# nichmorgan/better-search-rag-rust

Hardware: AMD Instinct MI355X
Metric: queries/sec + p50 latency, 768-d top-10 over N vectors @1/2/4/8 GPU (higher is better)
Workload: dtype f32; 1 GPU; configs[2]: 10M x 768 f32 corpus sharded over the N GPUs, 1000 batched queries, top-10; rows_total=10000000, rows_per_gpu_rank0=10000000, queries=1000, top_k=10, dim=768, parallelism=corpus sharded over 1 GPU(s) (interval_by_rank)

## Files before the change

### better-search-rag-rust_amd/csrc/index.cpp

```cpp
#include <math.h>
#include <stdio.h>
#include <string.h>
#include <time.h>

#include <algorithm>

#include "internal.hpp"
#include "kernels.hpp"

namespace bsr {

constexpr uint32_t kMaxKForFilter = 200;

static thread_local std::string g_err;

int set_error(int code, const char* fmt, ...) {
    char buf[1024];
    va_list ap;
    va_start(ap, fmt);
    vsnprintf(buf, sizeof buf, fmt, ap);
    va_end(ap);
    g_err = buf;
    return code;
}
// ... 632 lines not shown
                (unsigned long long)live, (unsigned long long)first, t1 - t0, t2 - t1, host_ms() - t2);
    return BSR_OK;
}

int bsr_index_compact_impl(bsr_index* ix, uint64_t new_global_offset, uint32_t flags, uint64_t* out_old_ids,
                           uint64_t out_capacity, uint64_t* out_count) {
    if (!ix) return set_error(BSR_E_INVALID, "null index");
    return ix->compact_rows(new_global_offset, flags, out_old_ids, out_capacity, out_count);
}

static int run_exact_scan(bsr_index* ix, const int32_t* ids, uint32_t n_ids, uint32_t k) {
    if (!n_ids) return BSR_OK;
    const uint32_t groups = (n_ids + kScanQF - 1) / kScanQF;
    const uint32_t grid = scan_grid_for(ix->n);
    BSR_TRY(ix->part.ensure((size_t)grid * kScanQF * k * sizeof(uint64_t)));
    ev_begin(ix, ix->ev_scan, 1);
    for (uint32_t g = 0; g < groups; ++g) {
        const uint32_t nqf = std::min(kScanQF, n_ids - g * kScanQF);
        const int32_t* qid = ids + (size_t)g * kScanQF;
        BSR_HIP(launch_scan_exact(ix->rows.as<float>(), ix->ld, ix->dim, ix->n, ix->na.as<float>(),
                                  ix->qf32.as<float>(), qid, nqf, ix->nb.as<float>(), k, grid,
                                  ix->part.as<uint64_t>(), ix->stream));
        BSR_HIP(launch_merge_parts(ix->part.as<uint64_t>(), grid, qid, nqf, k, ix->keys.as<uint64_t>(), ix->stream));
    }
    ev_end(ix, ix->ev_scan);
    return BSR_OK;
}

static int run_list_scan(bsr_index* ix, const int32_t* ids, uint32_t n_ids, uint32_t k, const uint32_t* list,
                         uint32_t n_list);
static int run_exact_rounds(bsr_index* ix, const int32_t* ids, uint32_t n_ids, uint32_t k) {
    if (!ix->n_dead) return run_exact_scan(ix, ids, n_ids, k);
    BSR_TRY(ix->ensure_live_list());
    return run_list_scan(ix, ids, n_ids, k, ix->live_list.as<uint32_t>(), (uint32_t)ix->live_rows());
}

static uint32_t top_slots(const bsr_index* ix, uint32_t nq, uint32_t k) {
    const char* v = getenv("BSR_SKINNY_TOP");
    if (v && v[0] == '0') return 0;
    if (nq > kSkinnyMaxQ || ix->n < kSkinnyTopMinRows || kp_for(k) > 63 || k > 64 || ix->op_row_bytes > 16 * 64 ||
        ix->ld % 64 != 0 || ix->ld > 1024 || !rescore_kp_enabled())
        return 0;
    const uint32_t slots = 4 * skinny_top_lists((uint32_t)ix->n);
    return slots <= 64u * kTopKeysPerLane ? slots : 0;
}

static int filter_buffers(bsr_index* ix, uint32_t nq, uint32_t qpad, uint32_t k, uint32_t cap_in = 0) {
    const uint32_t kp = kp_for(k);
    const uint32_t cap = std::max(cap_in ? cap_in : cap_for(k), top_slots(ix, nq, k));
    ix->stats.n_candidates = kp;
    BSR_TRY(ix->tau.ensure((size_t)qpad * sizeof(float)));
    BSR_TRY(ix->cand.ensure((size_t)qpad * cap * sizeof(uint64_t)));
    BSR_TRY(ix->cnt.ensure(((size_t)qpad + 8 * kTailCounters + kGangWords) * sizeof(uint32_t)));
    BSR_TRY(ix->cand_rows.ensure((size_t)nq * kp * sizeof(uint32_t)));
    BSR_TRY(ix->ncand.ensure((size_t)nq * sizeof(uint32_t)));
    BSR_TRY(ix->tau_excl.ensure((size_t)nq * sizeof(float)));
    BSR_TRY(ix->fail.ensure((size_t)nq * sizeof(uint32_t)));
    BSR_TRY(ix->fail2.ensure((size_t)nq * sizeof(uint32_t)));
    return BSR_OK;
}

static GemmArgs gemm_args(bsr_index* ix, uint32_t qpad) {
    GemmArgs g{};
    g.A = ix->fop.as<uint8_t>();
    g.B = ix->qop.as<uint8_t>();
    g.row_bytes = ix->op_row_bytes;
    g.n_qt = qpad / kFilterTile;
    g.a_scale = ix->ascale.as<float>();
    g.b_scale = ix->qscale.as<float>();
    return g;
}
static GemmArgs emit_args(bsr_index* ix, uint32_t nq, uint32_t qpad) {
    GemmArgs g = gemm_args(ix, qpad);
    g.a_stride = ix->op_row_bytes;
    g.a_scale_rows = kQuantBlock;
    g.n_rows = (uint32_t)ix->n;
    g.n_rt = (uint32_t)((ix->n + kFilterTile - 1) / kFilterTile);
    g.cand = ix->cand.as<uint64_t>();
    g.cnt = ix->cnt.as<uint32_t>();
    g.n_q = nq;
    return g;
}

struct SampleLayout {
    uint32_t n_s, n_rt_s;
    bool compact;
    uint32_t tiles;
    uint32_t s_ld, n_vals;
};
static bool sample_tiles_on() {
    const char* v = getenv("BSR_SAMPLE_TILES");
    return !(v && v[0] == '0');
}
static SampleLayout sample_layout(const bsr_index* ix, uint32_t nq, uint32_t ks) {
    SampleLayout L{};
    const uint32_t BM = kFilterTile;
    L.n_s = (uint32_t)((ix->n + kSampleStride - 1) / kSampleStride);
    L.n_rt_s = (L.n_s + BM - 1) / BM;
    L.compact = L.n_s >= 32u * 8u * ks;
    const uint32_t nk = ix->op_row_bytes / 64;
    const bool qs16 = ix->op_row_bytes % 64 == 0 && nk % 2 == 0 && nk >= 2 && nk <= 12;
    if (L.compact && nq > kSkinnyMaxQ && qs16 && sample_tiles_on()) L.tiles = sample_tiles_for(ix->n);
    if (L.tiles) {
        const uint64_t last0 = ((uint64_t)(L.tiles - 1) * kSampleTileEvery + kSampleTilePhase) * 128;
        const uint64_t valid = std::min<uint64_t>(128, ix->n - last0);
        L.s_ld = 4 * L.tiles;
        L.n_vals = 4 * (L.tiles - 1) + (uint32_t)((valid + kQuantBlock - 1) / kQuantBlock);
    } else {
        L.s_ld = L.compact ? L.n_rt_s * (BM / 32) : L.n_rt_s * BM;
        L.n_vals = L.compact ? (L.n_s + 31) / 32 : L.n_s;
    }
    return L;
}

static int sample_pass(bsr_index* ix, uint32_t nq, uint32_t qpad, uint32_t k, uint64_t* smax, uint32_t ks_in = 0,
                       uint32_t cap_in = 0, const uint32_t* ks_q = nullptr) {
    BSR_TRY(filter_buffers(ix, nq, qpad, k, cap_in));
    ix->smp_tiles = 0;
    const bool skinny = nq <= kSkinnyMaxQ;
    const uint32_t cap = cap_in ? cap_in : cap_for(k);
    const uint32_t ks = ks_in ? ks_in : ks_for(k);
    const uint64_t n = ix->n;
    GemmArgs g = gemm_args(ix, qpad);
    uint32_t* status = ix->d_status;
    if (n > cap) {
        const SampleLayout L = sample_layout(ix, nq, ks);
        const uint32_t s_ld = L.s_ld, n_vals = L.n_vals;
        BSR_TRY(ix->S.ensure((size_t)qpad * s_ld * sizeof(float)));
        g.a_stride = ix->op_row_bytes;
        if (L.tiles) {
            g.a_scale_rows = kQuantBlock;
            g.n_rows = (uint32_t)n;
            g.n_rt = L.tiles;
            g.s_tiles = L.tiles;
            g.s_vals = n_vals;
            ix->smp_tiles = L.tiles;
            ix->smp_ld = s_ld;
            ix->smp_vals = n_vals;
        } else {
            g.A = ix->fop_s.as<uint8_t>();
            g.a_scale = ix->ascale_s.as<float>();
            g.a_scale_rows = kSampleScaleRows;
            g.n_rows = L.n_s;
            g.n_rt = L.n_rt_s;
        }
        g.S = ix->S.as<float>();
        g.s_ld = s_ld;
        g.s_compact = L.compact ? 1u : 0u;
        BSR_HIP(launch_timed(ix, ix->ev_sample, [&] {
            return skinny ? launch_filter_skinny_sample(g, ix->stream) : launch_filter_sample(g, ix->stream);
        }, 2));
        BSR_HIP(launch_select_tau(ix->S.as<float>(), s_ld, n_vals, nq, qpad, ix->qflags.as<uint32_t>(), ks,
                                  ix->tau.as<float>(), ix->cnt.as<uint32_t>(), status, ix->stream, smax, ks_q));
    } else {
        BSR_HIP(launch_select_tau(nullptr, 0, 0, nq, qpad, ix->qflags.as<uint32_t>(), ks, ix->tau.as<float>(),
                                  ix->cnt.as<uint32_t>(), status, ix->stream, smax, ks_q));
    }
    return BSR_OK;
}

static int emit_pass(bsr_index* ix, uint32_t nq, uint32_t qpad, uint32_t k, uint32_t cap_in = 0) {
    const bool skinny = nq <= kSkinnyMaxQ;
    GemmArgs g = emit_args(ix, nq, qpad);
    g.tau = ix->tau.as<float>();
    g.cap = cap_in ? cap_in : cap_for(k);
    g.tail = g.n_qt <= kTailCounters ? ix->cnt.as<uint32_t>() + qpad : nullptr;
    g.s_tiles = skinny ? 0u : ix->smp_tiles;
    g.S = ix->S.as<float>();
    g.s_ld = ix->smp_ld;
    g.s_vals = ix->smp_vals;
    BSR_HIP(launch_timed(ix, ix->ev_emit, [&] {
        hipError_t r = skinny ? launch_filter_skinny_emit(g, ix->stream) : launch_filter_emit(g, ix->stream);
        if (r == hipSuccess && g.s_tiles) r = launch_sample_fixup(g, ix->stream);
        return r;
    }));
    return BSR_OK;
}

static uint32_t top_layout_lab() {
    const char* lay = getenv("BSR_TOP_LAYOUT");
    return lay && lay[0] == '0' ? 0u : 2u;
}

static int top_pass(bsr_index* ix, uint32_t nq, uint32_t qpad, uint32_t k, uint32_t top) {
    BSR_TRY(filter_buffers(ix, nq, qpad, k));
    GemmArgs g = emit_args(ix, nq, qpad);
    g.cap = top;
    g.status = ix->d_status;
// ... 892 lines not shown
```

### better-search-rag-rust_amd/csrc/internal.hpp

```cpp
#pragma once

#include <hip/hip_runtime.h>
#include <stdarg.h>
#include <stdint.h>

#include <atomic>

#include <string>
#include <vector>

#include "bsr.h"
#include "kernels.hpp"

namespace bsr {

int set_error(int code, const char* fmt, ...);
void clear_error();

#define BSR_HIP(call)                                                                       \
    do {                                                                                    \
        hipError_t e_ = (call);                                                             \
        if (e_ != hipSuccess)                                                               \
            return ::bsr::set_error(BSR_E_HIP, "%s failed: %s (%s:%d)", #call,              \
                                    hipGetErrorString(e_), __FILE__, __LINE__);             \
// ... 5 lines not shown
        if (r_ != BSR_OK) return r_; \
    } while (0)

extern std::atomic<uint64_t> g_alloc_gen;

struct DevBuf {
    void* p = nullptr;
    size_t bytes = 0;
    int ensure(size_t need);
    void release();
    template <class T> T* as() const { return static_cast<T*>(p); }
    ~DevBuf() { release(); }
};

bool is_device_ptr(const void* p);
void* coherent_host_alias(const void* p);
hipError_t stream_wait(hipStream_t s);
hipError_t flag_wait(const uint32_t* flag, hipStream_t s);
int select_device(int device);

static inline uint64_t round_up(uint64_t x, uint64_t m) { return (x + m - 1) / m * m; }

struct Events {
    hipEvent_t a = nullptr, b = nullptr;
    bool armed = false;
    ~Events();
    int create();
};

}

struct bsr_index {
    bsr_config cfg{};
    int device = 0;
    hipStream_t stream = nullptr;
    uint32_t dim = 0, ld = 0;
    uint64_t n = 0, n_pad = 0, global_offset = 0;
    bool loaded = false;
    bool approx_ok = false;
    uint32_t row_flags = 0;
    uint32_t op_row_bytes = 0;
    float row_ebound = 0.0f;

    bsr::DevBuf rows;
    bsr::DevBuf na;
    bsr::DevBuf fop;
    bsr::DevBuf fop_s;
    bsr::DevBuf ascale_s;
    uint32_t smp_tiles = 0, smp_ld = 0, smp_vals = 0;
    bsr::DevBuf ascale;
    bsr::DevBuf flags;

    bsr::DevBuf q_in, qf32, nb, qop, qscale, ebound, qflags, tau, S, cand, cnt, cand_rows, ncand,
        tau_excl, keys, fail, fail2, part, qids, qids_id, tmp;

    bsr::DevBuf res[2];
    uint8_t* h_res = nullptr;
    uint8_t* h_res_dev = nullptr;
    size_t h_res_bytes = 0;
    uint32_t* h_flag = nullptr;
    uint32_t* h_flag_dev = nullptr;
    bsr::DevBuf pub_ticket;
    uint32_t cur = 0;
    bool next_status_clean = false;
    size_t res_off_cnt = 0, res_off_dist = 0, res_off_idx = 0, res_off_x = 0, res_bytes = 0;
    uint32_t* d_status = nullptr;
    uint32_t* d_cnt = nullptr;
    float* d_dist = nullptr;
    uint64_t* d_idx = nullptr;
    float* d_x = nullptr;

    std::vector<uint32_t> h_qflags, h_fail;

    bsr_search_stats stats{};
    bsr_profile prof{};
    bsr::Events ev_emit, ev_sample, ev_select, ev_rescore, ev_scan, ev_total;
    int prof_level = 2;

    struct SearchKey {
        uint32_t nq = 0, k = 0;
        const float* qsrc = nullptr;
        uint64_t n = 0, gen = 0;
        uint64_t dead_gen = 0;
        bool top = false;
        uint32_t top_layout = 2;
        bool skinny_glds = true;
        bool sample_tiles = true;
        bool operator==(const SearchKey& o) const {
            return nq == o.nq && k == o.k && qsrc == o.qsrc && n == o.n && gen == o.gen &&
                   dead_gen == o.dead_gen && top == o.top &&
                   top_layout == o.top_layout && skinny_glds == o.skinny_glds && sample_tiles == o.sample_tiles;
        }
    };
    struct SearchGraph {
        hipGraphExec_t exec = nullptr;
        SearchKey key;
    };
    bool capturing = false;
    SearchGraph graphs[2];
    SearchKey warm;
    uint64_t graph_replays = 0;
    ~bsr_index();

    int search_device(const float* queries, uint32_t nq, uint32_t k, int (*after_launch)(void*) = nullptr,
                      void* ctx = nullptr, bool force_threshold = false);
    int prepare_result(uint32_t nq, uint32_t k);

// ... 60 lines not shown
```

### better-search-rag-rust_amd/csrc/k_filter.hip

```cpp
#include <cstdlib>
#include "bsr_device.hpp"
#include "kernels.hpp"

#include <hip/hip_ext.h>

#include <limits.h>
#include <math.h>

#include <algorithm>
#include <type_traits>
#include <utility>

namespace bsr {

typedef __attribute__((ext_vector_type(4))) int i32x4_t;
typedef __attribute__((ext_vector_type(16))) int i32x16_t;
typedef __attribute__((address_space(3))) void lds_void_t;

constexpr int kSlots = 4;
constexpr int kSliceB = 64;
constexpr int kWCap = 256;
constexpr int kThreads = 512;

__device__ __forceinline__ void wait_vm0() { asm volatile("s_waitcnt vmcnt(0)" ::: "memory"); }
// ... 267 lines not shown
                    }
                }
            }
            if (stored) wait_vm0();
            kt = 0;
            ++ti;
        } else {
            ++kt;
        }
    }
    if constexpr (EMIT) {
        const uint32_t ecount = eq[kWCap - 1];
        const uint32_t ne = ecount < (uint32_t)(kWCap - 1) ? ecount : (uint32_t)(kWCap - 1);
        for (uint32_t i = lane; i < ne; i += kWave) {
            const uint32_t q = qt * BN + eq[i];
            const uint32_t gp = atomicAdd(p.cnt + q, 1u);
            if (gp < p.cap) p.cand[(uint64_t)q * p.cap + gp] = ekeys[i];
        }
    }
}

__device__ __forceinline__ void qs_barrier(uint32_t n) {
#define BSR_QS_WAIT(N) \
    case N: asm volatile("s_waitcnt vmcnt(" #N ") lgkmcnt(0)\n\ts_barrier" ::: "memory"); break;
    switch (n) {
        BSR_QS_WAIT(15) BSR_QS_WAIT(14) BSR_QS_WAIT(13) BSR_QS_WAIT(12) BSR_QS_WAIT(11) BSR_QS_WAIT(10)
        BSR_QS_WAIT(9) BSR_QS_WAIT(8) BSR_QS_WAIT(7) BSR_QS_WAIT(6) BSR_QS_WAIT(5) BSR_QS_WAIT(4)
        BSR_QS_WAIT(3) BSR_QS_WAIT(2) BSR_QS_WAIT(1)
        default: asm volatile("s_waitcnt vmcnt(0) lgkmcnt(0)\n\ts_barrier" ::: "memory"); break;
    }
#undef BSR_QS_WAIT
}
template <int N>
__device__ __forceinline__ void qs_wait() {
    asm volatile("s_waitcnt vmcnt(%0)\n\ts_barrier" ::"n"(N) : "memory");
}
__device__ __forceinline__ void qs_wait_n(int n) {
#define BSR_QS_N(N) \
    case N: qs_wait<N>(); break;
    switch (n) {
        BSR_QS_N(1) BSR_QS_N(2) BSR_QS_N(3) BSR_QS_N(4) BSR_QS_N(5) BSR_QS_N(6) BSR_QS_N(7) BSR_QS_N(8)
        BSR_QS_N(9) BSR_QS_N(10) BSR_QS_N(11) BSR_QS_N(12) BSR_QS_N(13) BSR_QS_N(14) BSR_QS_N(15)
        default: qs_wait<0>(); break;
    }
#undef BSR_QS_N
}

#ifdef BSR_FILTER_STAMPS
__device__ __forceinline__ void qs_vm_n(int n) {
#define BSR_QS_V(N) \
    case N: asm volatile("s_waitcnt vmcnt(" #N ")" ::: "memory"); break;
    switch (n) {
        BSR_QS_V(1) BSR_QS_V(2) BSR_QS_V(3) BSR_QS_V(4) BSR_QS_V(5) BSR_QS_V(6) BSR_QS_V(7) BSR_QS_V(8)
        default: asm volatile("s_waitcnt vmcnt(0)" ::: "memory"); break;
    }
#undef BSR_QS_V
}
#endif
typedef __attribute__((ext_vector_type(4))) int i32x4v_t;

template <class F, int... I>
__device__ __forceinline__ void static_for(std::integer_sequence<int, I...>, F&& f) {
    (f(std::integral_constant<int, I>{}), ...);
}

constexpr int kSampleTilesPerWG = 8;

__device__ __forceinline__ uint32_t qs16_swz(uint32_t row) { return ((row >> 3) & 1u) * 2u; }

#ifdef BSR_FILTER_COUNTERS
__device__ unsigned long long g_filter_counters[8];
extern "C" int bsr_lab_filter_counters(unsigned long long* out, int reset) {
    hipError_t e = hipMemcpyFromSymbol(out, HIP_SYMBOL(g_filter_counters), sizeof(g_filter_counters));
    if (e == hipSuccess && reset) {
        static const unsigned long long z[8] = {};
        e = hipMemcpyToSymbol(HIP_SYMBOL(g_filter_counters), z, sizeof(z));
    }
    return (int)e;
}
__device__ unsigned long long g_filter_wg_stamps[4096 * 9];
__device__ uint32_t g_lab_xcd_xor;
extern "C" int bsr_lab_set_xcd_xor(uint32_t v) {
    return (int)hipMemcpyToSymbol(HIP_SYMBOL(g_lab_xcd_xor), &v, sizeof v);
}
__device__ unsigned int g_filter_wg_tiles[4096 * 2];
extern "C" int bsr_lab_filter_wg_tiles(unsigned int* out) {
    return (int)hipMemcpyFromSymbol(out, HIP_SYMBOL(g_filter_wg_tiles), sizeof(g_filter_wg_tiles));
}
extern "C" int bsr_lab_filter_wg_stamps(unsigned long long* out) {
    return (int)hipMemcpyFromSymbol(out, HIP_SYMBOL(g_filter_wg_stamps), sizeof(g_filter_wg_stamps));
}
#define BSR_FCNT(I_) ++fcnt[I_]
#else
#define BSR_FCNT(I_) \
    do {             \
    } while (0)
#endif
#ifdef BSR_FILTER_STAMPS
__device__ unsigned long long g_filter_stamps[8];
extern "C" int bsr_lab_filter_stamps(unsigned long long* out, int reset) {
    hipError_t e = hipMemcpyFromSymbol(out, HIP_SYMBOL(g_filter_stamps), sizeof(g_filter_stamps));
    if (e == hipSuccess && reset) {
        static const unsigned long long z[8] = {};
        e = hipMemcpyToSymbol(HIP_SYMBOL(g_filter_stamps), z, sizeof(z));
    }
    return (int)e;
}
#define BSR_FST(V_)                                                                     \
    do {                                                                                \
        __builtin_amdgcn_sched_barrier(0);                                              \
        asm volatile("s_memtime %0\n\ts_waitcnt lgkmcnt(0)" : "=s"(V_)::"memory");       \
        __builtin_amdgcn_sched_barrier(0);                                              \
    } while (0)
#endif
template <bool EMIT, int NK, bool GANGS = true>
__global__ __launch_bounds__(512, 1) void k_filter_qs16(GemmArgs p) {
    constexpr int GANG = GANGS ? 2 : 0;
    constexpr bool L2 = !GANGS, FW = GANGS;
    constexpr int S = 8, A = 6;
    constexpr int kWaitN = A - 4, kYoung = A - 4, kClaimUse = ((A - 4) % 2 == 0 ? A - 3 : A - 2) + 1;
    constexpr int BM = 128, BN = kFilterTile, NT = 512, SLOT = BM * kSliceB;
    constexpr int CAP = 10;
    static_assert(NK % 2 == 0 && NK >= 2 && NK <= 12, "even slice counts up to 768 bytes");
    constexpr bool QUEUE = GANGS && EMIT && NK == 12;
    constexpr int QD = kEmitQueueDepth, REC_B = 144, HDR_B = 32, QW_BYTES = QD * (REC_B + HDR_B);
    static_assert(QD >= 1 && QD <= kWave, "the flush takes one record per lane");
    constexpr int EM_BYTES = QUEUE ? 8 * QW_BYTES + 2 * BN * 4 : EMIT ? NT * 2 * CAP * 8 : 0;
    static_assert(S * SLOT + EM_BYTES + 16 <= 160 * 1024, "the ring, the queues and the table fit one CU's LDS");
    constexpr int SB_BYTES = EMIT ? 0 : kSampleTilesPerWG * 4 * BN * 4;
    __shared__ __attribute__((aligned(1024))) uint8_t lds[S * SLOT + EM_BYTES + SB_BYTES + 16];
    float* const sbuf = reinterpret_cast<float*>(lds + S * SLOT + EM_BYTES);
    uint32_t* const lds_ids = reinterpret_cast<uint32_t*>(lds + S * SLOT + EM_BYTES + SB_BYTES);
    const int tid = threadIdx.x, lane = tid & 63, w = tid >> 6;
    const uint32_t wu = __builtin_amdgcn_readfirstlane(tid >> 6);
    uint64_t* const lkeys = reinterpret_cast<uint64_t*>(lds + S * SLOT) + tid;
    uint32_t ecnt[2] = {0, 0};

    const uint32_t b = blockIdx.x, xcd = b & 7, slot = b >> 3;
    const uint32_t G = (gridDim.x >> 3) / p.n_qt;
    const uint32_t n_phys = (p.n_rows + BM - 1) / BM;
    const uint32_t n_rt = !p.s_tiles ? n_phys : EMIT ? n_phys - p.s_tiles : p.s_tiles;
    auto phys = [&](uint32_t lt) -> uint32_t {
        if (!p.s_tiles) return lt;
        return EMIT ? lt + lt / (kSampleTileEvery - 1) : lt * kSampleTileEvery + kSampleTilePhase;
    };
    const bool active = slot < G * p.n_qt;
    const uint32_t qt = active ? slot % p.n_qt : 0;
#ifdef BSR_FILTER_COUNTERS
    const uint32_t g0 = (xcd ^ g_lab_xcd_xor) * G + (active ? slot / p.n_qt : 0);
#else
    const uint32_t g0 = xcd * G + (active ? slot / p.n_qt : 0);
#endif
    const uint32_t RG = 8 * G;
    const uint32_t my_rt = (active && g0 < n_rt) ? (n_rt - 1 - g0) / RG + 1 : 0;
    const uint32_t J = my_rt * NK;
    constexpr uint32_t kEnd = 0xFFFFFFFFu;
    constexpr bool kStaticSched = NK > A;
    const bool dyn = EMIT && kStaticSched && p.tail != nullptr && active;
    const uint32_t n_st = dyn ? n_rt - n_rt / kTailDiv : n_rt;
    const uint32_t my_static = (active && g0 < n_st) ? (n_st - 1 - g0) / RG + 1 : 0;
    const uint32_t n_tail = n_rt - n_st, pool_sz = (n_tail + 7) / 8;
    uint32_t cpool = xcd, pools_tried = 1;
    auto pool_n = [&](uint32_t x) -> uint32_t {
        const uint32_t lo = x * pool_sz;
        return lo >= n_tail ? 0u : min(pool_sz, n_tail - lo);
    };
    auto claim_raw = [&]() -> uint32_t {
        uint32_t z;
        asm volatile("v_mov_b32 %0, 0" : "=v"(z));
        return atomicAdd(p.tail + cpool * p.n_qt + qt + z, 1u);
    };
    auto tail_id = [&](uint32_t v) -> uint32_t {
        for (;;) {
            if (v < pool_n(cpool)) return n_st + cpool * pool_sz + v;
            if (pools_tried == 8) return kEnd;
            ++pools_tried;
            cpool = (cpool + 1) & 7;
            v = atomicAdd(p.tail + cpool * p.n_qt + qt, 1u);
        }
    };
    auto claim = [&]() -> uint32_t { return tail_id(claim_raw()); };
    const bool gang = GANG && EMIT && kStaticSched && active && p.tail != nullptr && p.n_qt >= 2 && p.n_qt <= 4 &&
                      my_static >= kGangMinTiles;
    unsigned long long* const gprog =
        reinterpret_cast<unsigned long long*>(p.tail + 8 * kTailCounters) + (gang ? g0 : 0u);
    auto gang_raw = [&]() -> unsigned long long {
        uint32_t z;
        asm volatile("v_mov_b32 %0, 0" : "=v"(z));
        return atomicAdd(gprog + z, 1ull << (16 * qt));
    };
    auto gang_throttle = [&](unsigned long long old) {
        const uint32_t me = (uint32_t)(old >> (16 * qt)) & 0xFFFFu;
        int lag = 0;
        for (uint32_t j = 0; j < p.n_qt; ++j)
            if (j != qt) lag = max(lag, (int)(int16_t)(uint16_t)(me - ((uint32_t)(old >> (16 * j)) & 0xFFFFu)));
        for (int i = GANG; i < lag && i < GANG + 4; ++i) __builtin_amdgcn_s_sleep(32);
    };

    uint32_t qq[2];
    i32x4v_t fb[2][NK];
    float tau[2], sbq[2];
#pragma unroll
    for (int nb = 0; nb < 2; ++nb) {
        qq[nb] = qt * BN + w * 32 + nb * 16 + (lane & 15);
        const uint8_t* src = p.B + (uint64_t)qq[nb] * p.row_bytes + 16 * (lane >> 4);
#pragma unroll
        for (int kt = 0; kt < NK; ++kt) fb[nb][kt] = *reinterpret_cast<const i32x4v_t*>(src + 64 * kt);
        tau[nb] = EMIT ? p.tau[qq[nb]] : 0.0f;
        sbq[nb] = p.b_scale[qq[nb]];
    }
    auto flush_ring = [&](int nb) {
// ... 82 lines not shown
    auto issue_dma = [&](uint32_t jj) {
        uint8_t* la = lds + (jj % S) * SLOT + wu * 1024;
        __builtin_amdgcn_raw_ptr_buffer_load_lds(rsrc_a, (lds_void_t*)la, 16, aoff_dma, iss_kt * kSliceB, 0, 0);
        if (++iss_kt == NK) {
            iss_kt = 0;
            ++iss_ti;
            if (iss_ti < my_rt) tile_src(iss_ti, rsrc_a, aoff_dma);
        }
    };
    const uint32_t aoff0 = (lane & 15) * kSliceB + (((lane >> 4) ^ qs16_swz(lane & 15)) * 16);
    i32x4v_t fa[4];
    auto read_frag = [&](uint32_t jj, int rb) {
        fa[rb & 3] = *reinterpret_cast<const i32x4v_t*>(lds + (jj % S) * SLOT + rb * 1024 + aoff0);
    };

    i32x4v_t acc[8][2];
    uint32_t cur_id = my_rt ? g0 : kEnd, nxt_id = my_rt > 1 ? g0 + RG : kEnd;
    if (dyn && my_static < 2) {
        if (tid == 0) {
            const uint32_t a0 = my_static ? g0 : claim();
            lds_ids[2] = a0;
            lds_ids[3] = a0 == kEnd ? kEnd : claim();
        }
        __syncthreads();
        cur_id = __builtin_amdgcn_readfirstlane(lds_ids[2]);
        nxt_id = __builtin_amdgcn_readfirstlane(lds_ids[3]);
    } else if (dyn) {
        cur_id = g0;
        nxt_id = g0 + RG;
    }
    const bool any_tile = cur_id != kEnd;
    const uint32_t pre = (dyn ? any_tile : J != 0) ? (uint32_t)A : 0u;
    if (any_tile) {
        tile_src_rt(cur_id, rsrc_a, aoff_dma);
        rs_cur = rsrc_a;
        off_cur = aoff_dma;
        tile_src_rt(nxt_id != kEnd ? nxt_id : cur_id, rs_nxt, off_nxt);
    }
    if (kStatic) {
        for (uint32_t jj = 0; jj < pre; ++jj) {
            uint8_t* la = lds + (jj % S) * SLOT + wu * 1024;
            __builtin_amdgcn_raw_ptr_buffer_load_lds(rs_cur, (lds_void_t*)la, 16, off_cur, jj * kSliceB, 0, 0);
        }
    } else {
        for (uint32_t jj = 0; jj < pre; ++jj) issue_dma(jj);
    }
    qs_barrier(pre >= 3 ? pre - 3 : 0);
    if (any_tile)
#pragma unroll
        for (int rb = 0; rb < 4; ++rb) read_frag(0, rb);

#ifdef BSR_FILTER_COUNTERS
    unsigned long long fcnt[5] = {0, 0, 0, 0, 0};
    if (EMIT && tid == 0 && blockIdx.x < 4096) g_filter_wg_stamps[blockIdx.x * 9] = __builtin_amdgcn_s_memrealtime();
#endif
#ifdef BSR_FILTER_STAMPS
    unsigned long long fst[8] = {0, 0, 0, 0, 0, 0, 0, 0}, st_a, st_b, st_loop0;
    BSR_FST(st_loop0);
#endif
    for (uint32_t t = 0; cur_id != kEnd; ++t) {
        const uint32_t rt = phys(cur_id);
        BSR_FCNT(4);
        if (kStatic && t) {
            rs_cur = rs_nxt;
            off_cur = off_nxt;
            tile_src_rt(nxt_id != kEnd ? nxt_id : cur_id, rs_nxt, off_nxt);
        }
        float4 scv = make_float4(1.0f, 1.0f, 1.0f, 1.0f);
        if (EMIT) scv = *reinterpret_cast<const float4*>(p.a_scale + (uint64_t)rt * (BM / kQuantBlock));
        uint32_t n2 = (t + 2 < my_static) ? g0 + (t + 2) * RG : kEnd;
        const bool req = dyn && t + 2 >= my_static && nxt_id != kEnd;
        uint32_t claimed = 0;
        if (req && tid == 0) claimed = claim_raw();
        const bool thr = gang && t + 2 < my_static;
        unsigned long long gold = 0;
        if (thr && tid == 0) gold = gang_raw();
        const int w0_req = ((req || thr) && w == 0) ? 1 : 0;
        float sc_tile = 1.0f, sc_blk[4] = {1.0f, 1.0f, 1.0f, 1.0f};
        if constexpr (!EMIT) {
            if (p.s_tiles) {
#pragma unroll
                for (int g = 0; g < 4; ++g) sc_blk[g] = p.a_scale[rt * (BM / kQuantBlock) + g];
            } else {
                sc_tile = p.a_scale[rt * BM / kSampleScaleRows];
#pragma unroll
                for (int g = 0; g < 4; ++g) sc_blk[g] = sc_tile;
            }
        }
        static_for(std::make_integer_sequence<int, NK>{}, [&](auto KT) {
            constexpr int kt = decltype(KT)::value;
            const uint32_t jj = t * NK + kt;
            const bool bar_slice = (kt & 1) == 1;
#pragma unroll
            for (int rb = 0; rb < 8; ++rb) {
#pragma unroll
                for (int nb = 0; nb < 2; ++nb) {
                    if (kt == 0) {
                        const i32x4v_t z = {};
                        acc[rb][nb] = __builtin_amdgcn_mfma_i32_16x16x64_i8(fa[rb & 3], fb[nb][kt], z, 0, 0, 0);
                    } else {
                        acc[rb][nb] = __builtin_amdgcn_mfma_i32_16x16x64_i8(fa[rb & 3], fb[nb][kt], acc[rb][nb], 0, 0, 0);
                    }
                }
                __builtin_amdgcn_sched_barrier(0);
                if (rb < 4) {
                    read_frag(jj, rb + 4);
                } else {
                    read_frag(jj + 1, rb - 4);
                }
                if (kt == kClaimUse && rb == 0 && req && tid == 0) lds_ids[t & 1] = tail_id(claimed);
                if (GANG && kt == kClaimUse && rb == 0 && thr && tid == 0) gang_throttle(gold);
                if (bar_slice ? rb == 6 : rb == 1) {
                    if (kStatic) dma_static(jj + A, kt);
                    else issue_dma(jj + A);
                }
                if (bar_slice && rb == 5 && (kStatic || jj + 1 < J)) {
#ifdef BSR_FILTER_STAMPS
                    if (EMIT) {
                        BSR_FST(st_a);
                        qs_vm_n(kWaitN + ((EMIT && kt <= kYoung) ? 1 + w0_req : 0));
                        BSR_FST(st_b);
                        fst[6] += st_b - st_a;
                        st_a = st_b;
                        asm volatile("s_barrier" ::: "memory");
                        BSR_FST(st_b);
                        fst[kt == 1 ? 3 : 4] += st_b - st_a;
                    } else
#endif
                    qs_wait_n(kWaitN + ((EMIT && kt <= kYoung) ? 1 + w0_req : 0));
                }
                __builtin_amdgcn_sched_barrier(0);
            }
        });
        const float sc[4] = {scv.x, scv.y, scv.z, scv.w};
        bool stored = false;
        if constexpr (!EMIT) {
            if (p.s_compact) {
                const bool part = p.s_tiles && rt * BM + BM > p.n_rows;
#pragma unroll
                for (int g = 0; g < 4; ++g)
#pragma unroll
                    for (int nb = 0; nb < 2; ++nb) {
                        i32x4v_t x = acc[2 * g][nb], y = acc[2 * g + 1][nb];
                        if (part) {
                            const uint32_t r0 = rt * BM + g * 32 + 4 * (lane >> 4);
#pragma unroll
                            for (int r = 0; r < 4; ++r) {
                                x[r] = r0 + r < p.n_rows ? x[r] : INT_MIN;
                                y[r] = r0 + 16 + r < p.n_rows ? y[r] : INT_MIN;
                            }
                        }
                        int m = max(max(max(x[0], x[1]), max(x[2], x[3])), max(max(y[0], y[1]), max(y[2], y[3])));
                        const auto p16 = __builtin_amdgcn_permlane16_swap(m, m, false, false);
                        m = max((int)p16[0], (int)p16[1]);
                        const auto p32 = __builtin_amdgcn_permlane32_swap(m, m, false, false);
                        m = max((int)p32[0], (int)p32[1]);
                        const float v = ((float)m * sc_blk[g]) * sbq[nb];
                        if (lane < 16) sbuf[((t % kSampleTilesPerWG) * 4 + g) * BN + (qq[nb] - qt * BN)] = v;
                    }
                if (t % kSampleTilesPerWG == kSampleTilesPerWG - 1 || t + 1 == my_rt) {
                    __syncthreads();
                    const uint32_t t0 = t - t % kSampleTilesPerWG, nt = t + 1 - t0;
                    for (uint32_t i = tid; i < nt * BN; i += NT) {
                        const uint32_t tt = i / BN, ql = i % BN;
                        const float4 v = make_float4(sbuf[(tt * 4 + 0) * BN + ql], sbuf[(tt * 4 + 1) * BN + ql],
                                                     sbuf[(tt * 4 + 2) * BN + ql], sbuf[(tt * 4 + 3) * BN + ql]);
                        *reinterpret_cast<float4*>(p.S + (uint64_t)(qt * BN + ql) * p.s_ld + (g0 + (t0 + tt) * RG) * 4) = v;
                    }
                    stored = true;
                }
            } else {
#pragma unroll
                for (int rb = 0; rb < 8; ++rb) {
                    const uint32_t rbase = rt * BM + rb * 16 + 4 * (lane >> 4);
#pragma unroll
                    for (int nb = 0; nb < 2; ++nb) {
                        const i32x4v_t& x = acc[rb][nb];
                        const float v0 = ((float)x[0] * sc_tile) * sbq[nb], v1 = ((float)x[1] * sc_tile) * sbq[nb];
                        const float v2 = ((float)x[2] * sc_tile) * sbq[nb], v3 = ((float)x[3] * sc_tile) * sbq[nb];
                        *reinterpret_cast<float4*>(p.S + (uint64_t)qq[nb] * p.s_ld + rbase) = make_float4(v0, v1, v2, v3);
                    }
                }
                stored = true;
            }
        } else {
            const float sc_hi = fmaxf(fmaxf(sc[0], sc[1]), fmaxf(sc[2], sc[3]));
            const float sc_lo = fminf(fminf(sc[0], sc[1]), fminf(sc[2], sc[3]));
            bool any = false;
            BSR_FCNT(0);
#ifdef BSR_FILTER_STAMPS
            BSR_FST(st_a);
            fst[7] += 1;
#endif
            int mrb[2];
            bool l1p[2];
#pragma unroll
            for (int nb = 0; nb < 2; ++nb) {
                int m = acc[0][nb][0];
#pragma unroll
                for (int rb = 0; rb < 8; ++rb)
#pragma unroll
                    for (int r = 0; r < 4; ++r) m = (rb | r) ? max(m, acc[rb][nb][r]) : m;
                mrb[nb] = m;
                l1p[nb] = ((float)m * (m >= 0 ? sc_hi : sc_lo)) * sbq[nb] >= tau[nb];
                any |= l1p[nb];
            }
            const bool l2 = __ballot(any) != 0;
#ifdef BSR_FILTER_STAMPS
            BSR_FST(st_b);
            fst[0] += st_b - st_a;
            st_a = st_b;
#endif
            if (l2) {
                BSR_FCNT(1);
                if constexpr (QUEUE) {
                    const uint64_t lbit = 1ull << lane;
#pragma unroll
                    for (int nb = 0; nb < 2; ++nb) {
                        uint64_t bal = __ballot(l1p[nb]);
                        while (bal) {
                            if (nrec == (uint32_t)QD) {
                                flush_queue();
                                stored = true;
                            }
                            const uint32_t rank =
                                __builtin_amdgcn_mbcnt_hi((uint32_t)(bal >> 32), __builtin_amdgcn_mbcnt_lo((uint32_t)bal, 0u));
                            const bool mine = (bal & lbit) && rank < (uint32_t)QD - nrec;
                            if (mine) {
                                const uint32_t sl = nrec + rank;
#pragma unroll
                                for (int rb = 0; rb < 8; ++rb)
                                    *reinterpret_cast<i32x4v_t*>(qrec + sl * REC_B + rb * 16) = acc[rb][nb];
// ... 5 lines not shown
                            }
                            const uint64_t took = __ballot(mine);
                            nrec += (uint32_t)__builtin_popcountll(took);
                            bal &= ~took;
                        }
                    }
                } else {
#pragma unroll
                    for (int nb = 0; nb < 2; ++nb) {
                        if (!__ballot(((float)mrb[nb] * (mrb[nb] >= 0 ? sc_hi : sc_lo)) * sbq[nb] >= tau[nb])) continue;
                        BSR_FCNT(2);
                        uint32_t pm = 0;
                        bool pass_rb[8];
#pragma unroll
                        for (int rb = 0; rb < 8; ++rb) {
                            const i32x4v_t& x = acc[rb][nb];
                            const int bm = max(max(x[0], x[1]), max(x[2], x[3]));
                            if constexpr (L2) pass_rb[rb] = ((float)bm * sc[rb >> 1]) * sbq[nb] >= tau[nb];
                            else pm |= (((float)bm * sc[rb >> 1]) * sbq[nb] >= tau[nb]) ? 1u << rb : 0u;
                        }
#pragma unroll
                        for (int rb = 0; rb < 8; ++rb) {
                            if (!__ballot(L2 ? pass_rb[rb] : ((pm >> rb) & 1u))) continue;
                            BSR_FCNT(3);
                            if (__ballot(ecnt[nb] > (uint32_t)(CAP - 4))) {
                                flush_ring(nb);
                                stored = true;
                            }
                            const i32x4v_t& x = acc[rb][nb];
                            const float scr = sc[rb >> 1];
#pragma unroll
                            for (int r = 0; r < 4; ++r) {
                                const float v = ((float)x[r] * scr) * sbq[nb];
                                const uint32_t row = rt * BM + rb * 16 + 4 * (lane >> 4) + r;
                                lkeys[(nb * CAP + ecnt[nb]) * NT] = score_key(v, row);
                                ecnt[nb] += (v >= tau[nb] && row < p.n_rows) ? 1u : 0u;
                            }
                        }
                    }
                }
#ifdef BSR_FILTER_STAMPS
                BSR_FST(st_b);
                fst[1] += st_b - st_a;
                fst[2] += 1;
#endif
            }
        }
        if (stored) wait_vm0();
        cur_id = nxt_id;
        nxt_id = req ? __builtin_amdgcn_readfirstlane(lds_ids[t & 1]) : n2;
    }
    wait_vm0();
#ifdef BSR_FILTER_STAMPS
    if (EMIT) {
        BSR_FST(st_b);
        fst[5] = st_b - st_loop0;
        if (lane == 0)
            for (int i = 0; i < 8; ++i) atomicAdd(&g_filter_stamps[i], fst[i]);
    }
#endif
    if constexpr (EMIT) {
        if constexpr (QUEUE) {
            flush_queue();
        } else {
            flush_ring(0);
            flush_ring(1);
        }
#ifdef BSR_FILTER_COUNTERS
        if (lane == 0) {
            for (int i = 0; i < 4; ++i) atomicAdd(&g_filter_counters[i], fcnt[i]);
            if (blockIdx.x < 4096) g_filter_wg_stamps[blockIdx.x * 9 + 1 + w] = __builtin_amdgcn_s_memrealtime();
            if (blockIdx.x < 4096 && w == 0) {
                g_filter_wg_tiles[blockIdx.x * 2] = (unsigned int)fcnt[4];
                g_filter_wg_tiles[blockIdx.x * 2 + 1] = my_static;
            }
        }
#endif
    }
}


__global__ __launch_bounds__(256) void k_sample_fixup(GemmArgs p) {
    constexpr int NKM = 12, U = 4;
    const uint32_t q = blockIdx.x;
    const float tq = p.tau[q];
    if (!(tq < INFINITY)) return;
    const int tid = threadIdx.x, lane = tid & 63;
    const uint32_t w0 = __builtin_amdgcn_readfirstlane(tid >> 6) * 64;
    const uint32_t c = lane & 3, rr = lane >> 2;
    const int nk = p.row_bytes / kSliceB;
    const float sbq = p.b_scale[q];
    i32x4_t fb[NKM];
#pragma unroll
    for (int s = 0; s < NKM; ++s)
        fb[s] = s < nk ? *reinterpret_cast<const i32x4_t*>(p.B + (uint64_t)q * p.row_bytes + s * kSliceB + c * 16)
                       : i32x4_t{0, 0, 0, 0};
    auto block = [&](uint32_t j) {
        const uint32_t r0 = ((j >> 2) * kSampleTileEvery + kSampleTilePhase) * 128 + (j & 3) * 32;
        const float sc = p.a_scale[r0 / kQuantBlock];
        i32x4_t fa[2][NKM];
#pragma unroll
        for (int h = 0; h < 2; ++h) {
            const uint8_t* a = p.A + (uint64_t)(r0 + 16 * h + rr) * p.a_stride + c * 16;
#pragma unroll
            for (int s = 0; s < NKM; ++s)
                if (s < nk) fa[h][s] = *reinterpret_cast<const i32x4_t*>(a + s * kSliceB);
        }
#pragma unroll
        for (int h = 0; h < 2; ++h) {
            int acc = 0;
#pragma unroll
            for (int s = 0; s < NKM; ++s)
                if (s < nk)
#pragma unroll
                    for (int e = 0; e < 4; ++e) acc = __builtin_amdgcn_sdot4(fa[h][s][e], fb[s][e], acc, false);
            acc += (int)xor_lane32<1>((uint32_t)acc);
            acc += (int)xor_lane32<2>((uint32_t)acc);
            const float v = ((float)acc * sc) * sbq;
            const uint32_t row = r0 + 16 * h + rr;
            const bool pass = c == 0 && v >= tq && row < p.n_rows;
            const uint64_t mk = __ballot(pass);
            if (mk) {
                uint32_t gp = 0;
                if (lane == 0) gp = atomicAdd(p.cnt + q, (uint32_t)__builtin_popcountll(mk));
                gp = __builtin_amdgcn_readfirstlane(gp);
                const uint32_t pos = gp + (uint32_t)__builtin_popcountll(mk & ((1ull << lane) - 1ull));
                if (pass && pos < p.cap) p.cand[(uint64_t)q * p.cap + pos] = score_key(v, row);
            }
        }
    };
    const float* srow = p.S + (uint64_t)q * p.s_ld;
// ... 837 lines not shown
```

### better-search-rag-rust_amd/csrc/kernels.hpp

```cpp
#pragma once

#include <hip/hip_runtime.h>
#include <stdint.h>

namespace bsr {

constexpr uint32_t kLdAlign = 64;
constexpr uint32_t kRowPad = 256;
constexpr uint32_t kScanQF = 8;
constexpr uint32_t kSampleStride = 32;
constexpr uint32_t kQuantBlock = 32;
constexpr uint32_t kSampleScaleRows = 128;
constexpr uint32_t kFilterTile = 256;

constexpr uint32_t kRowNonFinite = 1u;
constexpr uint32_t kRowNormOvf = 2u;
constexpr uint32_t kRowNormRange = 4u;

constexpr uint32_t kQueryNonFinite = 1u;
constexpr uint32_t kQueryNoApprox = 2u;

enum StatusWord : uint32_t { kStFail = 0, kStEmitted = 1, kStQueryFlags = 2, kStFail2 = 3, kStWords = 4 };

hipError_t launch_synth_uniform(float* out, uint64_t row0, uint64_t n_rows, uint32_t dim,
// ... 60 lines not shown
hipError_t launch_dead_zero_fop(const uint64_t* dead, uint64_t n, const uint32_t* dead_blk, uint32_t row_bytes,
                                uint8_t* fop, uint8_t* fop_s, const float* rows, uint32_t dim, const float* scales_s,
                                hipStream_t s);
hipError_t launch_dead_andnot(const uint64_t* allow, const uint64_t* dead, uint64_t n, uint64_t* out, hipStream_t s);

enum UpdCount : uint32_t { kUpdBadId = 0, kUpdDupId = 1, kUpdNonFinite = 2, kUpdSampleRows = 3, kUpdCounts = 4 };
hipError_t launch_upd_check(const uint64_t* ids, uint64_t n_ids, uint64_t lo, uint64_t n, const void* src,
                            uint32_t dim, bool bf16, uint64_t* touched, uint64_t* blocks, uint64_t* groups,
                            uint64_t* cnt, hipStream_t s);
hipError_t launch_upd_scatter(const uint64_t* ids, uint64_t n_ids, uint64_t lo, const void* src, uint32_t dim,
                              uint32_t ld, bool bf16, float* rows, hipStream_t s);
hipError_t launch_upd_row_norms(const float* rows, const uint64_t* ids, uint64_t n_ids, uint64_t lo, uint32_t dim,
                                uint32_t ld, float* na, uint32_t* flags, hipStream_t s);
hipError_t launch_upd_rows_to_i8(const float* rows, uint64_t n, uint32_t dim, uint32_t ld, int8_t* out, float* scales,
                                 uint32_t* ea_max, const uint32_t* list, const uint32_t* count, uint32_t cap,
                                 hipStream_t s);
hipError_t launch_upd_rows_to_i8_sample(const float* rows, uint64_t n, uint32_t dim, uint32_t ld, int8_t* out,
                                        float* scales, const uint32_t* list, const uint32_t* count, uint32_t cap,
                                        hipStream_t s);

hipError_t launch_compact_gather(const float* rows, const uint32_t* list, uint64_t cnt, uint32_t ld, float* out,
                                 hipStream_t s);
hipError_t launch_compact_ids(const uint32_t* list, uint64_t cnt, uint64_t lo, uint64_t* out, uint32_t* first,
                              hipStream_t s);

struct GemmArgs {
    const uint8_t* A;
    uint64_t a_stride;
    uint32_t n_rows;
    uint32_t a_scale_rows;
    const uint8_t* B;
    uint32_t row_bytes;
    uint32_t n_rt, n_qt;
    const float* a_scale;
    const float* b_scale;
    float* S;
    uint32_t s_ld;
    uint32_t s_compact;
    const float* tau;
    uint64_t* cand;
    uint32_t* cnt;
    uint32_t cap;
    uint32_t* tail;
    uint32_t* status;
    uint32_t n_q;
    uint32_t top_layout;
    uint32_t s_tiles, s_vals;
};
constexpr uint32_t kSampleTileEvery = 32;
constexpr uint32_t kSampleTilePhase = 31;
static inline uint32_t sample_tiles_for(uint64_t n) { return (uint32_t)(((n + 127) / 128) / kSampleTileEvery); }
constexpr uint32_t kTailDiv = 8;
constexpr uint32_t kTailCounters = 64;
constexpr uint32_t kGangWords = 2 * 256;
constexpr uint32_t kGangMinTiles = 600;
constexpr int kEmitQueueDepth = 48;
hipError_t launch_filter_sample(const GemmArgs& a, hipStream_t s);
hipError_t launch_filter_emit(const GemmArgs& a, hipStream_t s);
hipError_t launch_filter_emit_gang(const GemmArgs& a, hipStream_t s);
hipError_t launch_sample_fixup(const GemmArgs& a, hipStream_t s);
constexpr uint32_t kSkinnyMaxQ = 16;
hipError_t launch_filter_skinny_sample(const GemmArgs& a, hipStream_t s);
hipError_t launch_filter_skinny_emit(const GemmArgs& a, hipStream_t s);
hipError_t launch_filter_skinny_top(const GemmArgs& a, hipStream_t s);
uint32_t skinny_top_lists(uint32_t n_rows);
bool skinny_glds_on();
constexpr uint64_t kSkinnyTopMinRows = 2u << 20;

hipError_t launch_select_tau(const float* S, uint32_t s_ld, uint32_t n_s, uint32_t nq,
                             uint32_t qpad, const uint32_t* qflags, uint32_t ks, float* tau,
                             uint32_t* cnt, uint32_t* status, hipStream_t s, uint64_t* smax = nullptr,
                             const uint32_t* ks_q = nullptr);
hipError_t launch_global_tau(const uint64_t* g, uint32_t P, uint32_t qpad, uint32_t nq, uint32_t ks,
                             const uint32_t* qflags, float* tau, hipStream_t s);
hipError_t launch_select_cand(const uint64_t* cand, const uint32_t* cnt, uint32_t cap,
                              uint32_t nq, const float* tau, uint32_t kp, uint32_t* cand_rows,
                              uint32_t* ncand, float* tau_excl, hipStream_t s);

struct RescoreArgs {
    const float* rows;
    uint32_t ld, dim;
    const float* na;
    const float* qf32;
    const float* nb;
    uint32_t n_items;
    const uint32_t* n_items_dev;
    const uint32_t* qlist;
    const uint32_t* cand_rows;
    const uint32_t* ncand;
    uint32_t kp;
    const float* tau_excl;
    const uint64_t* cand_keys;
    const uint32_t* cnt;
    uint32_t cap;
    const float* tau0;
    uint32_t sel;
    uint32_t top_w;
    const uint32_t* qflags;
    float* top_tau;
    uint32_t* top_cnt;
    uint32_t k;
    const float* ebound;
    uint64_t* out_keys;
    uint32_t* fail_cnt;
    uint32_t* fail_list;
    uint64_t* res_idx;
// ... 91 lines not shown
```

Measured before the change: 174,900 queries/s.

## Enable dynamic tail scheduling and per-wave compact stores in sample filter kernel

Extends the dynamic tail work-claiming scheme, previously used only by the emit filter, to the sampling pass. A dedicated tail counter buffer is added and reset by the last workgroup to finish, which is meant to reduce load imbalance at the end of the sample pass. The per-block max reduction is rewritten to merge the four row groups with paired permlane swaps. Sample results are stored per wave, keyed by the tile ids it processed, which removes a workgroup-wide barrier before the write-out. Scale loads are issued earlier and folded into the vmcnt wait accounting, which adds complexity and depends on the last-workgroup reset being correct.

```diff
diff --git a/better-search-rag-rust_amd/csrc/index.cpp b/better-search-rag-rust_amd/csrc/index.cpp
--- a/better-search-rag-rust_amd/csrc/index.cpp
+++ b/better-search-rag-rust_amd/csrc/index.cpp
@@ -708,6 +708,10 @@
     BSR_TRY(ix->tau.ensure((size_t)qpad * sizeof(float)));
     BSR_TRY(ix->cand.ensure((size_t)qpad * cap * sizeof(uint64_t)));
     BSR_TRY(ix->cnt.ensure(((size_t)qpad + 8 * kTailCounters + kGangWords) * sizeof(uint32_t)));
+    if (!ix->stail.p) {
+        BSR_TRY(ix->stail.ensure(kSampleTailWords * sizeof(uint32_t)));
+        BSR_HIP(hipMemsetAsync(ix->stail.p, 0, kSampleTailWords * sizeof(uint32_t), ix->stream));
+    }
     BSR_TRY(ix->cand_rows.ensure((size_t)nq * kp * sizeof(uint32_t)));
     BSR_TRY(ix->ncand.ensure((size_t)nq * sizeof(uint32_t)));
     BSR_TRY(ix->tau_excl.ensure((size_t)nq * sizeof(float)));
@@ -790,6 +794,7 @@
             g.n_rt = L.tiles;
             g.s_tiles = L.tiles;
             g.s_vals = n_vals;
+            g.tail = g.n_qt <= kTailCounters ? ix->stail.as<uint32_t>() : nullptr;
             ix->smp_tiles = L.tiles;
             ix->smp_ld = s_ld;
             ix->smp_vals = n_vals;
diff --git a/better-search-rag-rust_amd/csrc/internal.hpp b/better-search-rag-rust_amd/csrc/internal.hpp
--- a/better-search-rag-rust_amd/csrc/internal.hpp
+++ b/better-search-rag-rust_amd/csrc/internal.hpp
@@ -81,7 +81,7 @@
     bsr::DevBuf flags;
 
     bsr::DevBuf q_in, qf32, nb, qop, qscale, ebound, qflags, tau, S, cand, cnt, cand_rows, ncand,
-        tau_excl, keys, fail, fail2, part, qids, qids_id, tmp;
+        tau_excl, keys, fail, fail2, part, qids, qids_id, tmp, stail;
 
     bsr::DevBuf res[2];
     uint8_t* h_res = nullptr;
diff --git a/better-search-rag-rust_amd/csrc/k_filter.hip b/better-search-rag-rust_amd/csrc/k_filter.hip
--- a/better-search-rag-rust_amd/csrc/k_filter.hip
+++ b/better-search-rag-rust_amd/csrc/k_filter.hip
@@ -343,12 +343,14 @@
     case N: asm volatile("s_waitcnt vmcnt(" #N ")" ::: "memory"); break;
     switch (n) {
         BSR_QS_V(1) BSR_QS_V(2) BSR_QS_V(3) BSR_QS_V(4) BSR_QS_V(5) BSR_QS_V(6) BSR_QS_V(7) BSR_QS_V(8)
+        BSR_QS_V(9) BSR_QS_V(10) BSR_QS_V(11) BSR_QS_V(12) BSR_QS_V(13) BSR_QS_V(14) BSR_QS_V(15)
         default: asm volatile("s_waitcnt vmcnt(0)" ::: "memory"); break;
     }
 #undef BSR_QS_V
 }
 #endif
 typedef __attribute__((ext_vector_type(4))) int i32x4v_t;
+typedef __attribute__((ext_vector_type(4))) float f32x4v_t;
 
 template <class F, int... I>
 __device__ __forceinline__ void static_for(std::integer_sequence<int, I...>, F&& f) {
@@ -408,6 +410,11 @@
 __global__ __launch_bounds__(512, 1) void k_filter_qs16(GemmArgs p) {
     constexpr int GANG = GANGS ? 2 : 0;
     constexpr bool L2 = !GANGS, FW = GANGS;
+#ifdef BSR_STAMP_SAMPLE
+    [[maybe_unused]] constexpr bool kStamped = !EMIT;
+#else
+    [[maybe_unused]] constexpr bool kStamped = EMIT;
+#endif
     constexpr int S = 8, A = 6;
     constexpr int kWaitN = A - 4, kYoung = A - 4, kClaimUse = ((A - 4) % 2 == 0 ? A - 3 : A - 2) + 1;
     constexpr int BM = 128, BN = kFilterTile, NT = 512, SLOT = BM * kSliceB;
@@ -419,11 +426,13 @@
     constexpr int EM_BYTES = QUEUE ? 8 * QW_BYTES + 2 * BN * 4 : EMIT ? NT * 2 * CAP * 8 : 0;
     static_assert(S * SLOT + EM_BYTES + 16 <= 160 * 1024, "the ring, the queues and the table fit one CU's LDS");
     constexpr int SB_BYTES = EMIT ? 0 : kSampleTilesPerWG * 4 * BN * 4;
-    __shared__ __attribute__((aligned(1024))) uint8_t lds[S * SLOT + EM_BYTES + SB_BYTES + 16];
+    constexpr int SID_BYTES = EMIT ? 0 : 8 * kSampleTilesPerWG * 4;
+    __shared__ __attribute__((aligned(1024))) uint8_t lds[S * SLOT + EM_BYTES + SB_BYTES + SID_BYTES + 16];
     float* const sbuf = reinterpret_cast<float*>(lds + S * SLOT + EM_BYTES);
-    uint32_t* const lds_ids = reinterpret_cast<uint32_t*>(lds + S * SLOT + EM_BYTES + SB_BYTES);
+    uint32_t* const lds_ids = reinterpret_cast<uint32_t*>(lds + S * SLOT + EM_BYTES + SB_BYTES + SID_BYTES);
     const int tid = threadIdx.x, lane = tid & 63, w = tid >> 6;
     const uint32_t wu = __builtin_amdgcn_readfirstlane(tid >> 6);
+    uint32_t* const sids = reinterpret_cast<uint32_t*>(lds + S * SLOT + EM_BYTES + SB_BYTES) + wu * kSampleTilesPerWG;
     uint64_t* const lkeys = reinterpret_cast<uint64_t*>(lds + S * SLOT) + tid;
     uint32_t ecnt[2] = {0, 0};
 
@@ -447,7 +456,7 @@
     const uint32_t J = my_rt * NK;
     constexpr uint32_t kEnd = 0xFFFFFFFFu;
     constexpr bool kStaticSched = NK > A;
-    const bool dyn = EMIT && kStaticSched && p.tail != nullptr && active;
+    const bool dyn = kStaticSched && p.tail != nullptr && active;
     const uint32_t n_st = dyn ? n_rt - n_rt / kTailDiv : n_rt;
     const uint32_t my_static = (active && g0 < n_st) ? (n_st - 1 - g0) / RG + 1 : 0;
     const uint32_t n_tail = n_rt - n_st, pool_sz = (n_tail + 7) / 8;
@@ -636,7 +645,7 @@
 
 #ifdef BSR_FILTER_COUNTERS
     unsigned long long fcnt[5] = {0, 0, 0, 0, 0};
-    if (EMIT && tid == 0 && blockIdx.x < 4096) g_filter_wg_stamps[blockIdx.x * 9] = __builtin_amdgcn_s_memrealtime();
+    if (kStamped && tid == 0 && blockIdx.x < 4096) g_filter_wg_stamps[blockIdx.x * 9] = __builtin_amdgcn_s_memrealtime();
 #endif
 #ifdef BSR_FILTER_STAMPS
     unsigned long long fst[8] = {0, 0, 0, 0, 0, 0, 0, 0}, st_a, st_b, st_loop0;
@@ -651,7 +660,13 @@
             tile_src_rt(nxt_id != kEnd ? nxt_id : cur_id, rs_nxt, off_nxt);
         }
         float4 scv = make_float4(1.0f, 1.0f, 1.0f, 1.0f);
-        if (EMIT) scv = *reinterpret_cast<const float4*>(p.a_scale + (uint64_t)rt * (BM / kQuantBlock));
+        constexpr int kScaleLoads = EMIT ? 1 : 4;
+        if constexpr (EMIT) {
+            scv = *reinterpret_cast<const float4*>(p.a_scale + (uint64_t)rt * (BM / kQuantBlock));
+        } else {
+            const uint32_t s0 = p.s_tiles ? rt * (BM / kQuantBlock) : rt * BM / kSampleScaleRows, ds = p.s_tiles ? 1u : 0u;
+            scv = make_float4(p.a_scale[s0], p.a_scale[s0 + ds], p.a_scale[s0 + 2 * ds], p.a_scale[s0 + 3 * ds]);
+        }
         uint32_t n2 = (t + 2 < my_static) ? g0 + (t + 2) * RG : kEnd;
         const bool req = dyn && t + 2 >= my_static && nxt_id != kEnd;
         uint32_t claimed = 0;
@@ -660,17 +675,6 @@
         unsigned long long gold = 0;
         if (thr && tid == 0) gold = gang_raw();
         const int w0_req = ((req || thr) && w == 0) ? 1 : 0;
-        float sc_tile = 1.0f, sc_blk[4] = {1.0f, 1.0f, 1.0f, 1.0f};
-        if constexpr (!EMIT) {
-            if (p.s_tiles) {
-#pragma unroll
-                for (int g = 0; g < 4; ++g) sc_blk[g] = p.a_scale[rt * (BM / kQuantBlock) + g];
-            } else {
-                sc_tile = p.a_scale[rt * BM / kSampleScaleRows];
-#pragma unroll
-                for (int g = 0; g < 4; ++g) sc_blk[g] = sc_tile;
-            }
-        }
         static_for(std::make_integer_sequence<int, NK>{}, [&](auto KT) {
             constexpr int kt = decltype(KT)::value;
             const uint32_t jj = t * NK + kt;
@@ -700,9 +704,9 @@
                 }
                 if (bar_slice && rb == 5 && (kStatic || jj + 1 < J)) {
 #ifdef BSR_FILTER_STAMPS
-                    if (EMIT) {
+                    if (kStamped) {
                         BSR_FST(st_a);
-                        qs_vm_n(kWaitN + ((EMIT && kt <= kYoung) ? 1 + w0_req : 0));
+                        qs_vm_n(kWaitN + (kt <= kYoung ? kScaleLoads + w0_req : 0));
                         BSR_FST(st_b);
                         fst[6] += st_b - st_a;
                         st_a = st_b;
@@ -711,7 +715,7 @@
                         fst[kt == 1 ? 3 : 4] += st_b - st_a;
                     } else
 #endif
-                    qs_wait_n(kWaitN + ((EMIT && kt <= kYoung) ? 1 + w0_req : 0));
+                    qs_wait_n(kWaitN + (kt <= kYoung ? kScaleLoads + w0_req : 0));
                 }
                 __builtin_amdgcn_sched_barrier(0);
             }
@@ -721,37 +725,54 @@
         if constexpr (!EMIT) {
             if (p.s_compact) {
                 const bool part = p.s_tiles && rt * BM + BM > p.n_rows;
-#pragma unroll
-                for (int g = 0; g < 4; ++g)
-#pragma unroll
-                    for (int nb = 0; nb < 2; ++nb) {
-                        i32x4v_t x = acc[2 * g][nb], y = acc[2 * g + 1][nb];
-                        if (part) {
-                            const uint32_t r0 = rt * BM + g * 32 + 4 * (lane >> 4);
-#pragma unroll
-                            for (int r = 0; r < 4; ++r) {
-                                x[r] = r0 + r < p.n_rows ? x[r] : INT_MIN;
-                                y[r] = r0 + 16 + r < p.n_rows ? y[r] : INT_MIN;
-                            }
-                        }
-                        int m = max(max(max(x[0], x[1]), max(x[2], x[3])), max(max(y[0], y[1]), max(y[2], y[3])));
-                        const auto p16 = __builtin_amdgcn_permlane16_swap(m, m, false, false);
-                        m = max((int)p16[0], (int)p16[1]);
-                        const auto p32 = __builtin_amdgcn_permlane32_swap(m, m, false, false);
-                        m = max((int)p32[0], (int)p32[1]);
-                        const float v = ((float)m * sc_blk[g]) * sbq[nb];
-                        if (lane < 16) sbuf[((t % kSampleTilesPerWG) * 4 + g) * BN + (qq[nb] - qt * BN)] = v;
+                const uint32_t ts = t % kSampleTilesPerWG;
+#ifdef BSR_FILTER_STAMPS
+                if (kStamped) {
+                    BSR_FST(st_a);
+                    fst[7] += 1;
+                }
+#endif
+                const uint32_t vg = part ? (p.n_rows - rt * BM + 31) / 32 : 4u;
+                const uint32_t lg = lane >> 4;
+                const float scl = lg == 0 ? sc[0] : lg == 1 ? sc[1] : lg == 2 ? sc[2] : sc[3];
+#pragma unroll
+                for (int nb = 0; nb < 2; ++nb) {
+                    int m[4];
+#pragma unroll
+                    for (int g = 0; g < 4; ++g) {
+                        const i32x4v_t &x = acc[2 * g][nb], &y = acc[2 * g + 1][nb];
+                        m[g] = max(max(max(x[0], x[1]), max(x[2], x[3])), max(max(y[0], y[1]), max(y[2], y[3])));
+                        m[g] = (uint32_t)g < vg ? m[g] : INT_MIN;
                     }
-                if (t % kSampleTilesPerWG == kSampleTilesPerWG - 1 || t + 1 == my_rt) {
-                    __syncthreads();
-                    const uint32_t t0 = t - t % kSampleTilesPerWG, nt = t + 1 - t0;
-                    for (uint32_t i = tid; i < nt * BN; i += NT) {
-                        const uint32_t tt = i / BN, ql = i % BN;
-                        const float4 v = make_float4(sbuf[(tt * 4 + 0) * BN + ql], sbuf[(tt * 4 + 1) * BN + ql],
-                                                     sbuf[(tt * 4 + 2) * BN + ql], sbuf[(tt * 4 + 3) * BN + ql]);
-                        *reinterpret_cast<float4*>(p.S + (uint64_t)(qt * BN + ql) * p.s_ld + (g0 + (t0 + tt) * RG) * 4) = v;
+                    const auto s01 = __builtin_amdgcn_permlane16_swap(m[0], m[1], false, false);
+                    const int e = max((int)s01[0], (int)s01[1]);
+                    const auto s23 = __builtin_amdgcn_permlane16_swap(m[2], m[3], false, false);
+                    const int f = max((int)s23[0], (int)s23[1]);
+                    const auto s4 = __builtin_amdgcn_permlane32_swap(e, f, false, false);
+                    const int mg = max((int)s4[0], (int)s4[1]);
+                    const float v = ((float)mg * scl) * sbq[nb];
+                    sbuf[(ts * BN + (qq[nb] - qt * BN)) * 4 + lg] = v;
+                }
+#ifdef BSR_FILTER_STAMPS
+                if (kStamped) {
+                    BSR_FST(st_b);
+                    fst[0] += st_b - st_a;
+                    st_a = st_b;
+                }
+#endif
+                if (lane == 0) sids[ts] = cur_id;
+                if (ts == kSampleTilesPerWG - 1 || nxt_id == kEnd) {
+                    for (uint32_t i = lane; i < (ts + 1) * 32; i += kWave) {
+                        const uint32_t tt = i >> 5, ql = wu * 32 + (i & 31);
+                        const f32x4v_t v = *reinterpret_cast<const f32x4v_t*>(sbuf + (tt * BN + ql) * 4);
+                        *reinterpret_cast<f32x4v_t*>(p.S + (uint64_t)(qt * BN + ql) * p.s_ld + sids[tt] * 4) = v;
                     }
-                    stored = true;
+#ifdef BSR_FILTER_STAMPS
+                    if (kStamped) {
+                        BSR_FST(st_b);
+                        fst[1] += st_b - st_a;
+                    }
+#endif
                 }
             } else {
 #pragma unroll
@@ -760,8 +781,8 @@
 #pragma unroll
                     for (int nb = 0; nb < 2; ++nb) {
                         const i32x4v_t& x = acc[rb][nb];
-                        const float v0 = ((float)x[0] * sc_tile) * sbq[nb], v1 = ((float)x[1] * sc_tile) * sbq[nb];
-                        const float v2 = ((float)x[2] * sc_tile) * sbq[nb], v3 = ((float)x[3] * sc_tile) * sbq[nb];
+                        const float v0 = ((float)x[0] * sc[0]) * sbq[nb], v1 = ((float)x[1] * sc[0]) * sbq[nb];
+                        const float v2 = ((float)x[2] * sc[0]) * sbq[nb], v3 = ((float)x[3] * sc[0]) * sbq[nb];
                         *reinterpret_cast<float4*>(p.S + (uint64_t)qq[nb] * p.s_ld + rbase) = make_float4(v0, v1, v2, v3);
                     }
                 }
@@ -873,7 +894,7 @@
     }
     wait_vm0();
 #ifdef BSR_FILTER_STAMPS
-    if (EMIT) {
+    if (kStamped) {
         BSR_FST(st_b);
         fst[5] = st_b - st_loop0;
         if (lane == 0)
@@ -887,7 +908,14 @@
             flush_ring(0);
             flush_ring(1);
         }
+    } else if (kStaticSched && p.tail != nullptr && w == 0) {
+        uint32_t last = 0;
+        if (lane == 0) last = atomicAdd(p.tail + 8 * p.n_qt, 1u) == gridDim.x - 1 ? 1u : 0u;
+        if (__builtin_amdgcn_readfirstlane(last))
+            for (uint32_t i = lane; i <= 8 * p.n_qt; i += kWave) atomicExch(p.tail + i, 0u);
+    }
 #ifdef BSR_FILTER_COUNTERS
+    if (kStamped) {
         if (lane == 0) {
             for (int i = 0; i < 4; ++i) atomicAdd(&g_filter_counters[i], fcnt[i]);
             if (blockIdx.x < 4096) g_filter_wg_stamps[blockIdx.x * 9 + 1 + w] = __builtin_amdgcn_s_memrealtime();
@@ -896,8 +924,8 @@
                 g_filter_wg_tiles[blockIdx.x * 2 + 1] = my_static;
             }
         }
+    }
 #endif
-    }
 }
 
 
diff --git a/better-search-rag-rust_amd/csrc/kernels.hpp b/better-search-rag-rust_amd/csrc/kernels.hpp
--- a/better-search-rag-rust_amd/csrc/kernels.hpp
+++ b/better-search-rag-rust_amd/csrc/kernels.hpp
@@ -136,6 +136,7 @@
 static inline uint32_t sample_tiles_for(uint64_t n) { return (uint32_t)(((n + 127) / 128) / kSampleTileEvery); }
 constexpr uint32_t kTailDiv = 8;
 constexpr uint32_t kTailCounters = 64;
+constexpr uint32_t kSampleTailWords = 8 * kTailCounters + 1;
 constexpr uint32_t kGangWords = 2 * 256;
 constexpr uint32_t kGangMinTiles = 600;
 constexpr int kEmitQueueDepth = 48;
```

Measured after the change: 175,600 queries/s (median of 6 runs). Within noise of the previous version (+0.4%).
